# rosielab/emojivoice

Hardware: AMD Instinct MI355X
Metric: audio_seconds_per_second (higher is better)
Workload: dtype f32 (deep layers: operand = two block-scaled fp16 pieces, product = 3 fp16 products on the fp16 MFMA, f32 accumulate); 1 GPU; config2: batch 64 x 516-frame (5.99 s) utterances per GPU, 10 Euler steps + HiFi-GAN V1, 22.05 kHz; global_batch=64, frames=516, ode_steps=10, parallelism=dp1, collective=none, batch_pipeline=cfm(i+1) || hifigan(i) on two streams, 2 pipeline(s) in flight

## Files before the change

emojivoice_amd/_lib.py:

```python
from __future__ import annotations

import ctypes as C
import math
import os
import subprocess
from typing import Dict, Optional

import numpy as np
import torch

_HERE = os.path.dirname(os.path.abspath(__file__))
LIB_PATH = os.environ.get("EV_LIB_PATH") or os.path.join(_HERE, "lib", "libemojivoice_hip.so")
CSRC = os.path.join(_HERE, "csrc")
SOURCES = [os.path.join(CSRC, n) for n in ("ev_engine.hip", "ev_kernels.h", "ev_analysis_kernels.h", "ev_analysis.h")] \
    + [os.path.join(os.path.dirname(_HERE), "include", "emojivoice.h")]

EXPORTS = [
    "ev_abi_version", "ev_create", "ev_destroy", "ev_last_error", "ev_load_estimator", "ev_load_vocoder", "ev_load_vocoder_cfg", "ev_load_text_encoder", "ev_text_encoder",
    "ev_text_encoder_status", "ev_stft_magnitude", "ev_denoise", "ev_align", "ev_dbg_conv_bench",
    "ev_workspace_bytes", "ev_cfm_decode", "ev_estimator", "ev_hifigan", "ev_profile_enable", "ev_profile_read", "ev_profile_read_split", "ev_dbg_last_cfg", "ev_set_arithmetic", "ev_get_arithmetic",
    "ev_op_conv1d", "ev_op_groupnorm_mish", "ev_op_groupnorm_mish2", "ev_op_conv_groupnorm", "ev_op_layernorm", "ev_op_split_pieces", "ev_op_attention", "ev_op_ln_mlp", "ev_set_mrf_streams_max",
    "ev_cfm_decode2", "ev_reserve", "ev_alloc_count", "ev_dbg_sk_stats", "ev_op_attn_out", "ev_dbg_set_amax", "ev_dbg_set_attn_h16", "ev_dbg_set_chain", "ev_dbg_sk_taken",
    "ev_load_mel_basis", "ev_mel_spectrogram",
    "ev_maximum_path", "ev_log_prior", "ev_mas_align",
    "ev_estimator_rows", "ev_cfm_loss",
    "ev_load_resampler", "ev_resample", "ev_mel_stats",
    "ev_trim_bounds", "ev_trim_apply",
    "ev_pitch_yin", "ev_dtw",
    "ev_loudness",
    "ev_pyin_observe", "ev_pyin_decode",
    "ev_op_attention2", "ev_op_attn_out2",
    "ev_load_stoi", "ev_stoi",
    "ev_load_stft_dist", "ev_stft_dist",
    "ev_load_voice_quality", "ev_voice_quality",
    "ev_load_formants", "ev_formants", "ev_formant_track",
    "ev_perturbation",
    "ev_load_harmonics", "ev_harmonics",
    "ev_functionals", "ev_modulation",
    "ev_load_auditory", "ev_auditory",
    "ev_load_srmr", "ev_srmr",
    "ev_load_speech_rate", "ev_speech_rate",
    "ev_load_envelope", "ev_envelope",
    "ev_load_phase_vocoder", "ev_phase_vocoder",
    "ev_op_conv1d_epi",
]


class EvLibraryError(RuntimeError):
    pass


class ev_tensor_index(C.Structure):
    _fields_ = [("name", C.c_char_p), ("offset", C.c_uint64), ("ndim", C.c_int32), ("shape", C.c_int64 * 4)]


# ... 118 lines not shown
    lib.ev_stft_dist.argtypes = [vp, vp, vp, vp, i32, i32, C.c_double, vp, vp, vp, vp]
    lib.ev_load_voice_quality.argtypes = [vp, vp, vp, i32, i32, i32, vp, vp, i32, i32, i32, vp, C.c_double]
    lib.ev_voice_quality.argtypes = [vp, vp, vp, i32, i32, C.c_double, vp, vp, vp, vp]
    lib.ev_load_formants.argtypes = [vp, vp, i32, i32, i32, C.c_double, C.c_double, C.c_double, i32]
    lib.ev_formants.argtypes = [vp, vp, vp, i32, i32, C.c_double, vp, vp, vp, vp]
    lib.ev_formant_track.argtypes = [vp, vp, vp, i32, i32, i32, i32, vp, C.c_double, C.c_double, C.c_double, vp, vp, vp, vp, vp]
    lib.ev_perturbation.argtypes = [vp, vp, vp, i32, i32, i32, vp, i32, i32, C.c_double, C.c_double, C.c_double, vp, vp, vp, vp]
    lib.ev_load_harmonics.argtypes = [vp, vp, vp, i32, i32, i32, C.c_double, i32, C.c_double, C.c_double, C.c_double]
    lib.ev_harmonics.argtypes = [vp, vp, vp, i32, i32, vp, vp, vp, i32, C.c_double, vp, vp, vp, vp]
    lib.ev_functionals.argtypes = [vp, vp, vp, vp, i32, i32, i32, vp, i32, vp, vp, vp]
    lib.ev_modulation.argtypes = [vp, vp, vp, vp, i32, i32, i32, C.c_double, C.c_double, i32, i32, C.c_double, vp, i32, vp, vp, vp, vp, vp, vp]
    lib.ev_load_auditory.argtypes = [vp, vp, vp, i32, i32, i32, vp, i32, vp, vp, i32, i32, i32, C.c_double]
    lib.ev_auditory.argtypes = [vp, vp, vp, i32, i32, C.c_double, vp, vp, vp, vp, vp]
    lib.ev_load_srmr.argtypes = [vp, vp, vp, vp, vp, vp, i32, i32, i32]
    lib.ev_srmr.argtypes = [vp, vp, vp, i32, i32, vp, vp, vp, vp, vp]
    lib.ev_load_speech_rate.argtypes = [vp, vp, i32, i32]
    lib.ev_speech_rate.argtypes = [vp, vp, vp, vp, i32, i32, C.c_double, C.c_double, C.c_double, C.c_double, i32, i32, vp, vp, vp, vp, vp]
    lib.ev_load_envelope.argtypes = [vp, vp, i32, i32, C.c_double, C.c_double, C.c_double, vp, i32]
    lib.ev_envelope.argtypes = [vp, vp, vp, vp, i32, i32, C.c_double, vp, vp, vp, vp]
    lib.ev_load_phase_vocoder.argtypes = [vp, vp, vp, i32]
    lib.ev_phase_vocoder.argtypes = [vp, vp, vp, i32, i32, C.c_double, vp, i32, vp, vp, vp, vp]
    lib.ev_maximum_path.argtypes = [vp, vp, vp, vp, i32, i32, i32, vp, vp, vp]
    lib.ev_log_prior.argtypes = [vp, vp, vp, i32, i32, i32, vp, vp]
    lib.ev_mas_align.argtypes = [vp, vp, vp, vp, vp, i32, i32, i32, vp, vp, vp, vp, vp]
    lib.ev_profile_enable.argtypes = [vp, i32]
    lib.ev_profile_read.argtypes = [vp, C.POINTER(C.c_double), C.POINTER(C.c_double), C.POINTER(C.c_int64), i32]
    lib.ev_profile_read_split.argtypes = [vp, C.POINTER(C.c_double), C.POINTER(C.c_double), C.POINTER(C.c_int64)]
    lib.ev_dbg_last_cfg.argtypes = [vp]
    lib.ev_set_arithmetic.argtypes = [vp, i32]
    lib.ev_get_arithmetic.argtypes = [vp]
    lib.ev_dbg_set_amax.argtypes = [vp, i32]
    lib.ev_dbg_set_attn_h16.argtypes = [vp, i32]
    lib.ev_dbg_set_chain.argtypes = [vp, i32]
    lib.ev_dbg_sk_taken.argtypes = [vp]
    lib.ev_dbg_sk_taken.restype = C.c_int64
    lib.ev_op_conv1d.argtypes = [vp, vp, vp, vp, i32, i32, i32, i32, i32, i32, i32, i32, i32, f32, vp, vp]
    lib.ev_op_conv1d_epi.argtypes = [vp, vp, vp, vp, i32, i32, i32, i32, i32, i32, i32, i32, i32, i32, C.POINTER(ev_conv_epi), vp, vp, vp, vp]
    lib.ev_op_groupnorm_mish.argtypes = [vp, vp, vp, vp, vp, i32, i32, i32, i32, vp, vp]
    lib.ev_op_groupnorm_mish2.argtypes = [vp, vp, vp, vp, vp, i32, i32, i32, i32, i32, vp, i32, vp, vp, vp]
    lib.ev_op_conv_groupnorm.argtypes = [vp, vp, vp, vp, i32, i32, i32, vp, vp, vp, i32, vp, vp, vp, vp, vp, C.POINTER(C.c_int), vp]
    lib.ev_op_layernorm.argtypes = [vp, vp, vp, vp, i32, i32, vp, vp]
    lib.ev_op_split_pieces.argtypes = [vp, vp, i32, vp, vp]
    lib.ev_op_attention.argtypes = [vp, vp, vp, i32, i32, i32, vp, vp]
    lib.ev_op_attn_out.argtypes = [vp, vp, vp, i32, i32, vp, vp, vp, vp]
    lib.ev_op_attention2.argtypes = [vp, vp, vp, i32, i32, i32, i32, i32, i32, vp, C.POINTER(C.c_int), vp]
    lib.ev_op_attn_out2.argtypes = [vp, vp, vp, i32, i32, i32, i32, vp, vp, f32, f32, f32, vp, C.POINTER(C.c_int), vp]
    lib.ev_op_ln_mlp.argtypes = [vp, vp, vp, vp, vp, vp, vp, vp, vp, vp, vp, i32, i32, i32, vp, vp]
    for n in EXPORTS:
        getattr(lib, n)
    _lib = lib
    return lib


def _stream_ptr() -> int:
    return int(torch.cuda.current_stream().cuda_stream)


def _ptr(t):
    return None if t is None else t.data_ptr()


class Engine:

    def __init__(self, device: int = 0, spk_emb_dim: int = 64, heads: int = 2):
        if not torch.cuda.is_available():
            raise EvLibraryError("no ROCm GPU visible: the EmojiVoice hot path has no CPU fallback")
# ... 781 lines not shown
        B, F, T = mel.shape
        assert F == 80
        wav = torch.empty((B, 1, T * 256), dtype=torch.float32, device=mel.device)
        per_utt = (T + 2 * self.voc_pad0) * self.voc_frame_bytes
        bmax = max(1, int((2**32 - 2**20) // per_utt))
        for b0 in range(0, B, bmax):
            b1 = min(B, b0 + bmax)
            self._check(self.lib.ev_hifigan(self.h, mel[b0:b1].data_ptr(), b1 - b0, T, wav[b0:b1].data_ptr(), _stream_ptr()), "ev_hifigan")
        return wav

    def workspace_bytes(self, B: int, Tp: int, Tv: int) -> int:
        return int(self.lib.ev_workspace_bytes(self.h, B, Tp, Tv))

    def profile_enable(self, on: bool):
        self._check(self.lib.ev_profile_enable(self.h, int(on)), "ev_profile_enable")

    def op_split_pieces(self, x):
        x = self._f32(x).reshape(-1)
        out = torch.empty((3, x.numel()), dtype=torch.float32, device=x.device)
        self._check(self.lib.ev_op_split_pieces(self.h, x.data_ptr(), x.numel(), out.data_ptr(), _stream_ptr()), "ev_op_split_pieces")
        return out

    def set_arithmetic(self, bf16_products: int):
        self._check(self.lib.ev_set_arithmetic(self.h, int(bf16_products)), "ev_set_arithmetic")

    def set_amax(self, on: bool) -> None:
        self._check(self.lib.ev_dbg_set_amax(self.h, int(bool(on))), "ev_dbg_set_amax")

    def set_attn_h16(self, on: bool) -> None:
        self._check(self.lib.ev_dbg_set_attn_h16(self.h, int(bool(on))), "ev_dbg_set_attn_h16")

    def set_chain(self, on: bool) -> None:
        self._check(self.lib.ev_dbg_set_chain(self.h, int(bool(on))), "ev_dbg_set_chain")

    def arithmetic(self) -> int:
        return int(self.lib.ev_get_arithmetic(self.h))

    def last_cfg(self) -> int:
        return int(self.lib.ev_dbg_last_cfg(self.h))

    def profile_read_split(self):
        ms, fl, n = C.c_double(), C.c_double(), C.c_int64()
        self._check(self.lib.ev_profile_read_split(self.h, C.byref(ms), C.byref(fl), C.byref(n)), "ev_profile_read_split")
        return ms.value, fl.value, n.value

    def profile_read(self, reset: bool = True):
        ms, fl, n = C.c_double(), C.c_double(), C.c_int64()
        self._check(self.lib.ev_profile_read(self.h, C.byref(ms), C.byref(fl), C.byref(n), int(reset)), "ev_profile_read")
        return ms.value, fl.value, n.value

    def op_conv1d(self, x, w, bias, dilation=1, transposed=False, stride=1, padding=0, pre_lrelu_slope=-1.0):
        x = self._f32(x)
        B, Cin, T = x.shape
        w = np.ascontiguousarray(w.detach().cpu().float().numpy())
        if transposed:
            Cout, K = w.shape[1], w.shape[2]
            Tout = T * stride
        else:
            Cout, K = w.shape[0], w.shape[2]
            Tout = T // stride
        bp = None
        if bias is not None:
            bnp = np.ascontiguousarray(bias.detach().cpu().float().numpy())
            bp = bnp.ctypes.data_as(C.c_void_p)
        y = torch.empty((B, Cout, Tout), dtype=torch.float32, device=x.device)
        self._check(self.lib.ev_op_conv1d(self.h, x.data_ptr(), w.ctypes.data_as(C.c_void_p), bp, B, Cin, T, Cout, K, dilation,
# ... 163 lines not shown
```

emojivoice_amd/csrc/ev_engine.hip:

```cpp
#include "ev_kernels.h"
#include "../../include/emojivoice.h"

#include <math.h>
#include <stdlib.h>
#include <stdarg.h>
#include <stdio.h>
#include <string.h>

#include <algorithm>
#include <atomic>
#include <mutex>
#include <numeric>
#include <string>
#include <unordered_map>
#include <vector>

namespace {

struct HostTensor {
    const float* p = nullptr;
    int ndim = 0;
    int64_t shape[4] = {0, 0, 0, 0};
    int64_t numel() const { int64_t n = 1; for (int i = 0; i < ndim; ++i) n *= shape[i]; return n; }
};
// ... 102 lines not shown
    ResamplerW rs;
    StoiW stoi;
    StftDistW stftd;
    VoiceQW voiceq;
    FormantW fmt;
    HarmW harm;
    AudW aud;
    SrmrW srmr;
    RateW rate;
    EnvW env;
    PvW pv;
    struct Scratch { char* p = nullptr; size_t bytes = 0; hipStream_t last = nullptr; bool last_valid = false; };
    Scratch dn_ws, enc_ws, mas_ws;
    Scratch dtw_ws;
    Scratch stat_ws;
    Scratch trim_ws;
    Scratch loud_ws;
    Scratch stoi_ws;
    Scratch stftd_ws;
    Scratch srmr_ws;
    Scratch rate_ws;
    Scratch env_ws;
    Scratch pv_ws;
    float* zeros = nullptr;
    int max_steps = 64;
    int* bad_ids_host = nullptr; int* bad_ids_dev = nullptr;
    char* ws = nullptr; size_t ws_bytes = 0; size_t ws_used = 0; size_t ws_bytes_last = 0;
    int ws_B = -1, ws_Tp = -1, ws_Tv = -1;
    bool prof = false;
    bool fuse_pairs = true;
    bool fuse_attn = true;
    bool attn_h16 = true;
    bool use_chain = true;
    bool fuse_mlp = true;
    int gn_stats_tiles = 0;
    int fuse_mlp_min_tiles = 96;
    std::vector<hipEvent_t> ev_pool; size_t ev_used = 0;
    hipStream_t ws_stream = nullptr; bool ws_stream_valid = false;
    float* temb_host[2] = {nullptr, nullptr}; size_t temb_cap[2] = {0, 0}; hipEvent_t temb_ev[2] = {nullptr, nullptr}; int temb_slot = 0;
    float* cap_pool = nullptr; size_t cap_stride = 0; int cap_used = 0; int cap_nt[8] = {0};
    struct TprojEntry { int nt; float* d; };
    std::vector<TprojEntry> tproj_cache;
    bool captured = false; int cap_B = 0, cap_Tp = 0;
    int64_t n_allocs = 0;
    double prof_flops = 0; int64_t prof_launches = 0;
    struct ProfRec { int kind, Cin, Cout, ntaps, nrows, cfg, lean; double flops; bool split = false; };
    std::vector<ProfRec> prof_recs;
    hipStream_t stream = nullptr;
    hipStream_t mrf_stream[2] = {nullptr, nullptr};
    hipEvent_t mrf_ev[4] = {nullptr, nullptr, nullptr, nullptr};
    int ncu = 0;
    unsigned* sk_ctrl = nullptr;
    unsigned sk_seq = 0;
    float* sk_part = nullptr;
    int split_terms = 16;
    bool use_amax = true;
    bool amax_emitted = false;
    int n_fp32_only_layers = 0;
    int last_cfg = -1;
    bool sk_balance = true;
    int sk_wgs = 2;
    int sk_spin = 3000;
    int mrf_max_frames = 16384;
    int force_cfg = -1;
    bool lean = true;
    bool small_sk = true;
// ... 805 lines not shown
    const ConvLayer& Lout = mode == 0 ? *L2 : L1;
    p.Y = Y; p.ldy = ldy; p.Cout = Lout.Cout; p.bias = mode == 0 ? Lout.bias : nullptr; p.osplit_log2 = 31; p.isplit_log2 = 31; p.mmul = 1;
    p.nrows = g.nrows; p.S = g.S; p.P = g.P; p.T = g.T; p.scale = 1.f;
    p.R = R; p.ldr = 256; p.rowmask = rowmask; p.mask2 = (mode == 0 && rowmask) ? 1 : 0;
    mp.X = X; mp.ldx = 256; mp.ln_g = ln_g; mp.ln_b = ln_b; mp.ln_eps = 1e-5f;
    if (!L1.bias && !h->zeros) {
        HIPCHK(h, hipMalloc((void**)&h->zeros, 4096 * sizeof(float)));
        HIPCHK(h, hipMemsetAsync(h->zeros, 0, 4096 * sizeof(float), h->stream));
        h->owned.push_back(h->zeros);
    }
    if (L1.Mpad > 4096) return fail(h, "launch_mlp: hidden width %d > 4096", L1.Mpad);
    mp.W1 = L1.W; mp.b1 = L1.bias ? L1.bias : h->zeros; mp.M1 = L1.Mpad; mp.alpha = alpha; mp.binv = binv; mp.W2 = L2 ? L2->W : nullptr;
    if (L1.Cin != 256 || L1.Kpad != 256 || L1.ntaps != 1 || (L1.Mpad % 128) || L1.Cout != L1.Mpad || (ldy & 3))
        return fail(h, "launch_mlp: first linear must be 256 -> multiple of 128 (got %d -> %d)", L1.Cin, L1.Cout);
    if (mode == 0 && (!L2 || L2->Cout != 256 || L2->Mpad != 256 || L2->Cin != L1.Cout || L2->Kpad != L1.Mpad || L2->ntaps != 1 || !L2->bias || !alpha || !binv))
        return fail(h, "launch_mlp: second linear must be %d -> 256 with bias", L1.Cout);
    if (over_4gib(g, std::max(ldy, 256))) return fail(h, "tensor exceeds the 4 GiB buffer-addressing limit: split the batch");
    if (g.S < 4 && g.nrows > 1) return fail(h, "launch_mlp: utterance stride %d < 4 rows is not supported by the lean row walk", g.S);
    const int nchunk = L1.Mpad / 128;
    const double flops = 2.0 * (L1.macs_per_row + (L2 ? L2->macs_per_row : 0.0)) * valid_rows(g);
    {
        const int split_terms = h->split_terms;
        const int nt64 = (g.nrows + 63) / 64;
        if (mode == 0 && (split_terms == 6 || split_terms == 16) && L1.Wx && L2->Wx && h->sk_balance && h->ncu > 0 && h->ncu <= EV_SK_MAXWG && nt64 >= h->ncu) {
            const int grid = h->ncu;
            const bool h16 = split_terms == 16 && L1.Wh && L2->Wh;
            mp.W1x = L1.Wx; mp.W2x = L2->Wx; mp.ntiles = nt64;
            mp.W1h = L1.Wh; mp.W2h = L2->Wh; mp.w1_scale = L1.wh_scale; mp.w2_scale = L2->wh_scale;
            if (sk_setup(h, mp.sk, (long)nt64 * nchunk, grid, h16)) return 1;
            if (L1.Mpad > 1024) return fail(h, "launch_mlp: hidden width %d > 1024 (LDS table of the SnakeBeta vectors)", L1.Mpad);
            const size_t smem = h16 ? (size_t)64 * (4 * 256 + 16) + (size_t)64 * (4 * 128 + 16) + 16 + (size_t)2 * L1.Mpad * sizeof(float) + 64
                                    : (size_t)64 * (6 * 256 + 16) + (size_t)64 * (6 * 128 + 16) + 16 + (size_t)2 * L1.Mpad * sizeof(float);
            if (prof_begin(h)) return 1;
            if (h16) launch<ln_mlp_h16_kernel<0>>(h->device, dim3(grid), dim3(256), smem, h->stream, mp);
            else launch<ln_mlp_split_kernel<6>>(h->device, dim3(grid), dim3(256), smem, h->stream, mp);
            HIPCHK(h, hipGetLastError());
            return h->prof ? prof_end(h, {2, 256, Lout.Cout, 1, g.nrows, h16 ? 121 : 120, 1, flops, true}) : 0;
        }
    }
    {
        const int nt64 = (g.nrows + 63) / 64;
        if (mode == 1 && h->split_terms == 16 && h->qkv_h16 && L1.Wh && L1.Mpad == 384 && !R && !rowmask && h->ncu > 0 && nt64 >= h->ncu) {
            mp.W1h = L1.Wh; mp.w1_scale = L1.wh_scale; mp.ntiles = nt64;
            if (qkv_scale && qkv_packed && qkv_scale[0] > 0.f && qkv_scale[1] > 0.f && qkv_scale[2] > 0.f) {
                mp.qkv_pack = 1; *qkv_packed = 1;
                for (int i = 0; i < 3; ++i) mp.qkv_scale[i] = qkv_scale[i];
            }
            const size_t smem = (size_t)64 * (4 * 256 + 16) + 32;
            if (prof_begin(h)) return 1;
            launch<ln_qkv_h16_kernel<0>>(h->device, dim3(nt64), dim3(256), smem, h->stream, mp);
            HIPCHK(h, hipGetLastError());
            h->last_cfg = 122;
            return h->prof ? prof_end(h, {3, 256, Lout.Cout, 1, g.nrows, 122, 1, flops, true}) : 0;
        }
    }
    const int ntiles = (g.nrows + 31) / 32;
    size_t smem = (size_t)(32 * 260 + 4 * 32 * 36 + 4) * sizeof(float);
    int grid = ntiles;
    mp.ntiles = ntiles;
    mp.sk.q = nchunk; mp.sk.r = 0; mp.sk.spin_limit = h->sk_spin;
    const int wpc = h->sk_wgs;
    const bool big = ntiles >= h->ncu && (long)ntiles * nchunk >= (long)wpc * h->ncu;
    if (h->sk_balance && h->ncu > 0 && wpc * h->ncu <= EV_SK_MAXWG && big) {
        const long U = (long)ntiles * nchunk;
        grid = (int)std::min<long>((long)wpc * h->ncu, U);
        if (sk_setup(h, mp.sk, U, grid, false)) return 1;
        if (wpc != 2) smem = std::max(smem, (size_t)((160 * 1024 / wpc) & ~255));
    }
    if (prof_begin(h)) return 1;
// ... 663 lines not shown
        constexpr int w = decltype(kernel_tag)::value;
        if (fused) launch<mas_search_kernel<w, true>>(h->device, dim3(B), dim3(NT), smem, st, p);
        else launch<mas_search_kernel<w, false>>(h->device, dim3(B), dim3(NT), smem, st, p);
    };
    dispatch<16, 4>(W, go);
    HIPCHK(h, hipGetLastError());
    if (d_attn || d_mu_y) {
        hipLaunchKernelGGL(mas_fill_kernel, dim3((Ty + 255) / 256, B, d_attn ? (Tx + 63) / 64 : 1), dim3(256), 0, st, (const int32_t*)p.idx, d_mu_x, d_attn, d_mu_y, C, Tx, Ty);
        HIPCHK(h, hipGetLastError());
    }
    return 0;
}

}

extern "C" {

int ev_abi_version(void) { return EV_ABI_VERSION; }

int ev_create(ev_handle** out, int device, const ev_model_dims* dims) {
    if (!out || !dims) return 1;
    *out = nullptr;
    int ndev = 0;
    if (hipGetDeviceCount(&ndev) != hipSuccess || device < 0 || device >= ndev) return 2;
    if (hipSetDevice(device) != hipSuccess) return 3;
    ev_handle* h = new ev_handle();
    h->device = device;
    h->dims = *dims;
    { const char* fp = getenv("EV_FUSE_PAIRS"); if (fp && *fp == '0') h->fuse_pairs = false; }
    { const char* fp = getenv("EV_FUSE_MLP"); if (fp && *fp == '0') h->fuse_mlp = false; }
    { const char* fp = getenv("EV_FUSE_ATTN"); if (fp && *fp == '0') h->fuse_attn = false; }
    if (getenv("EV_NO_ATTN_H16")) h->attn_h16 = false;
    if (getenv("EV_NO_CHAIN")) h->use_chain = false;
    { const char* fp = getenv("EV_FUSE_MLP_MIN"); if (fp && *fp) h->fuse_mlp_min_tiles = atoi(fp); }
    { const char* fp = getenv("EV_MRF_STREAMS_MAX"); if (fp && *fp) h->mrf_max_frames = atoi(fp); }
    if (getenv("EV_NO_AMAX")) h->use_amax = false;
    { const char* sp = getenv("EV_SPLIT"); if (sp && *sp) { const int t = atoi(sp); h->split_terms = (t == 0 || t == 3 || t == 6 || t == 9 || t == 16) ? t : 16; } }
    { const char* fp = getenv("EV_NO_SK_BALANCE"); if (fp && *fp && *fp != '0') h->sk_balance = false; }
    { const char* fp = getenv("EV_SK_SPIN"); if (fp && *fp) h->sk_spin = atoi(fp); }
    { const char* fp = getenv("EV_SK_WGS"); if (fp && *fp) h->sk_wgs = std::min(3, std::max(1, atoi(fp))); }
    { const char* fp = getenv("EV_FORCE_CFG"); if (fp && *fp) h->force_cfg = atoi(fp); }
    if (getenv("EV_NO_LEAN")) h->lean = false;
    if (getenv("EV_NO_SK")) h->small_sk = false;
    if (getenv("EV_NO_SK32_LEAN")) h->sk32_lean = false;
    if (getenv("EV_NO_GN_STATS")) h->gn_stats = false;
    if (getenv("EV_NO_QKV_H16")) h->qkv_h16 = false;
    if (getenv("EV_NO_ATTN_SK")) h->attn_sk = false;
    { const char* fp = getenv("EV_ATTN_TPW"); if (fp) h->attn_tpw = std::max(1, atoi(fp)); }
    if (getenv("EV_FULL_REZERO")) h->full_rezero = true;
    { const char* fp = getenv("EV_RB2_MINKEEP"); if (fp) h->rb2_minkeep = atoi(fp); }
    if (hipDeviceGetAttribute(&h->ncu, hipDeviceAttributeMultiprocessorCount, device) != hipSuccess) h->ncu = 0;
    if (dims->n_feats != 80 || dims->channels != 256 || dims->head_dim != 64 || dims->heads != 2) {
        delete h;
        return 4;
    }
    *out = h;
    return 0;
}

void ev_destroy(ev_handle* h) {
    if (!h) return;
    hipSetDevice(h->device);
    hipDeviceSynchronize();
    for (void* p : h->owned) hipFree(p);
    if (h->ws) hipFree(h->ws);
    if (h->cap_pool) hipHostFree(h->cap_pool);
// ... 942 lines not shown
    if (reset) { h->ev_used = 0; h->prof_flops = 0; h->prof_launches = 0; h->prof_recs.clear(); }
    return 0;
}

int ev_dbg_last_cfg(ev_handle* h) { return h ? h->last_cfg : -1; }

int ev_set_arithmetic(ev_handle* h, int bf16_products) {
    if (!h) return 1;
    if (bf16_products != 0 && bf16_products != 3 && bf16_products != 6 && bf16_products != 9 && bf16_products != 16)
        return fail(h, "ev_set_arithmetic: 0, 3, 6, 9 or 16, got %d", bf16_products);
    h->split_terms = bf16_products;
    return 0;
}
int ev_get_arithmetic(ev_handle* h) { return h ? h->split_terms : -1; }

int ev_dbg_set_amax(ev_handle* h, int on) {
    if (!h) return 1;
    h->use_amax = on != 0;
    return 0;
}

int ev_dbg_set_chain(ev_handle* h, int on) {
    if (!h) return 1;
    h->use_chain = on != 0;
    return 0;
}

int ev_dbg_set_attn_h16(ev_handle* h, int on) {
    if (!h) return 1;
    h->attn_h16 = on != 0;
    return 0;
}

int ev_profile_read_split(ev_handle* h, double* ms_out, double* flops_out, int64_t* launches_out) {
    if (!h) return 1;
    HIPCHK(h, hipStreamSynchronize(h->stream));
    double ms = 0, fl = 0;
    int64_t n = 0;
    if (h->prof_recs.size() * 2 == h->ev_used)
        for (size_t i = 0; i < h->prof_recs.size(); ++i) {
            const auto& r = h->prof_recs[i];
            if (!r.split) continue;
            float t = 0;
            HIPCHK(h, hipEventElapsedTime(&t, h->ev_pool[2 * i], h->ev_pool[2 * i + 1]));
            ms += t; fl += r.flops; n += 1;
        }
    if (ms_out) *ms_out = ms;
    if (flops_out) *flops_out = fl;
    if (launches_out) *launches_out = n;
    return 0;
}

int ev_dbg_conv_bench(ev_handle* h, int Cin, int Cout, int K, int dil, int B, int T, int P, int iters, int dbg, int cfg, float* ms_out) {
    const int stagger = (dbg & 64) ? 0 : -1;
    const bool planar = (dbg & 32) != 0;
    const bool no_res = (dbg & 128) != 0;
    const bool no_pro = (dbg & 512) != 0;
    dbg &= ~(64 | 32 | 128 | 512);
    if (enter(h)) return 1;
    h->stream = nullptr;
    std::vector<float> w((size_t)Cout * Cin * K), b(Cout);
    unsigned s = 12345u;
    for (auto& v : w) { s = s * 1664525u + 1013904223u; v = ((s >> 8) * (1.0f / 16777216.0f) - 0.5f) * 0.1f; }
    for (auto& v : b) { s = s * 1664525u + 1013904223u; v = ((s >> 8) * (1.0f / 16777216.0f) - 0.5f); }
    HostTensor wt, bt;
    wt.p = w.data(); wt.ndim = 3; wt.shape[0] = Cout; wt.shape[1] = Cin; wt.shape[2] = K;
// ... 500 lines not shown
```

emojivoice_amd/csrc/ev_kernels.h:

```cpp
#pragma once
#include <hip/hip_runtime.h>
#include <stdint.h>
#include <type_traits>

typedef float f32x16 __attribute__((ext_vector_type(16)));
typedef float f32x4 __attribute__((ext_vector_type(4)));
typedef int i32x4 __attribute__((ext_vector_type(4)));

#define EV_MAX_TAPS 16
#define EV_BK 32
#define EV_LDK 36
#define EV_WROWS 128
#define EV_SK_MAXF4(TW) ((TW) == 4 ? (64 + 64) * 8 * 8 : 16 * 512)
#define EV_HALO 64

enum { ACT_NONE = 0, ACT_LRELU = 1, ACT_TANH = 2, ACT_SILU = 3, ACT_MISH = 4, ACT_SNAKE = 5 };

struct SkCtl {
    unsigned* ctrl;
    unsigned* flags;
    float* part;
    int part_floats;
    int q, r;
    int spin_limit;
// ... 3977 lines not shown
            while (c1 < nchunk) {
                int n = 0;
                while (n < 64 && gi + n < (int)gridDim.x && sk_start(mp.sk, gi + n) < tile_end) ++n;
                if (n == 0) break;
                const int ready = sk_wait_many(mp.sk, gi, n, tag, tid, skw);
                for (int k = 0; k < ready; ++k) acc_io((unsigned)(gi + k) * pslot, 1);
                gi += ready;
                if (ready < n) {
                    const int sgi = sk_start(mp.sk, gi);
                    int egi = sk_start(mp.sk, gi + 1);
                    egi = egi < tile_end ? egi : tile_end;
                    acc_io((unsigned)g * pslot + pslot / 2, 0);
                    asm volatile("s_waitcnt vmcnt(0)" ::: "memory");
                    cA = sgi - t * nchunk; cB = egi - t * nchunk;
                    spilled = true; again = true;
                    ++gi;
                    break;
                }
            }
            if (again) {
                const int ht0 = cA * 4 + wave;
                ldP(R0, ht0, 0); ldP(R1, ht0, 1); ldP(R2, ht0, 2); ldP(R3, ht0, 3); ldP(R4, ht0, 4); ldP(R5, ht0, 5); ldP(R6, ht0, 6); ldP(R7, ht0, 7);
                continue;
            }
            conv_epilogue_lean<2, 2, 1>(p, acc2, smem + wave * (32 * 68), wave * 64, n0, lane);
            break;
        }
    }
    if (pend_pub) sk_publish(mp.sk, g, tag, tid);
    sk_arrive(mp.sk, tag, tid);
}

template <int UNUSED = 0>
__global__ __launch_bounds__(256, 2) void ln_qkv_h16_kernel(const MlpParams mp) {
    constexpr int NT = 64, C = 256, TM = 3;
    constexpr int XRS = 4 * C + 16;
    const ConvParams& p = mp.ep;
    extern __shared__ __attribute__((aligned(16))) float smem[];
    char* Xb = (char*)smem;
    float* red = (float*)(Xb + NT * XRS);
    const int tid = threadIdx.x, lane = tid & 63;
    const int wave = __builtin_amdgcn_readfirstlane(tid >> 6);
    const int li = lane & 31, lh = lane >> 5;
    const __amdgpu_buffer_rsrc_t rX = ev_rsrc(mp.X), rW1 = ev_rsrc(mp.W1h), rB1 = ev_rsrc(mp.b1);
    const unsigned wlane = (unsigned)lane * 16u;
    const int n0 = blockIdx.x * NT;
    if (ev_tile_is_padding(p.S, p.P, p.T, p.nrows, n0, NT)) return;
    f32x4 A[4][TM][2];
    auto ldA = [&](f32x4 (&dst)[TM][2], int sl) {
#pragma unroll
        for (int i = 0; i < TM; ++i)
#pragma unroll
            for (int pc = 0; pc < 2; ++pc) dst[i][pc] = ev_bload4(rW1, wlane, (unsigned)((((wave * TM + i) * (C / 16) + sl) * 2 + pc) * 1024));
    };
    ldA(A[0], 0); ldA(A[1], 1); ldA(A[2], 2);
    f32x4 bq[TM][4];
    const unsigned coff = (unsigned)(4 * lh) * 4u;
#pragma unroll
    for (int i = 0; i < TM; ++i)
#pragma unroll
        for (int q = 0; q < 4; ++q) bq[i][q] = ev_bload4(rB1, coff + (unsigned)((wave * TM + i) * 32 + 8 * q) * 4u, 0);
    float sx;
    {
        const f32x4 gm = *(const f32x4*)(mp.ln_g + lane * 4), be = *(const f32x4*)(mp.ln_b + lane * 4);
        f32x4 xv[16];
#pragma unroll
// ... 1562 lines not shown
```

include/emojivoice.h:

```cpp
#ifndef EMOJIVOICE_H
#define EMOJIVOICE_H

#include <stddef.h>
#include <stdint.h>

#ifdef __cplusplus
extern "C" {
#endif

#define EV_ABI_VERSION 4

typedef struct ev_handle ev_handle;

typedef struct ev_tensor_index {
    const char *name;
    uint64_t offset;
    int32_t ndim;
    int64_t shape[4];
} ev_tensor_index;

typedef struct ev_model_dims {
    int32_t n_feats;
    int32_t spk_emb_dim;
    int32_t channels;
// ... 173 lines not shown

int ev_functionals(ev_handle *h, const double *d_v , const uint8_t *d_mask ,
                   const int32_t *d_len , int B, int K, int F,
                   const double *q , int NQ,
                   double *d_stat , int32_t *d_count , void *stream);

int ev_modulation(ev_handle *h, const double *d_v , const uint8_t *d_mask ,
                  const int32_t *d_len , int B, int K, int F,
                  double nu0, double dnu, int NM, int min_run, double min_cycles,
                  const int32_t *band , int NBAND,
                  double *d_spec , int32_t *d_weight , double *d_peak ,
                  double *d_stat , int32_t *d_count , void *stream);

int ev_load_auditory(ev_handle *h, const double *window , const double *twiddle , int W, int H, int nfft,
                     const double *mel_w , int n_mel, const double *eq ,
                     const double *dct , int n_ceps, int k_lo, int k_hi, double compress );
int ev_auditory(ev_handle *h, const float *d_x , const int32_t *d_len , int B, int L, double power_floor,
                double *d_frame , double *d_mfcc , int32_t *d_flags ,
                double *d_bands , void *stream);

int ev_profile_enable(ev_handle *h, int on);
int ev_profile_read(ev_handle *h, double *conv_ms, double *conv_flops, int64_t *conv_launches, int reset);
int ev_profile_read_split(ev_handle *h, double *ms, double *flops, int64_t *launches);
int ev_set_arithmetic(ev_handle *h, int setting);
int ev_get_arithmetic(ev_handle *h);

int ev_dbg_last_cfg(ev_handle *h);

int ev_dbg_conv_bench(ev_handle *h, int Cin, int Cout, int K, int dil, int B, int T, int P, int iters, int dbg, int cfg, float *ms_out);

int ev_dbg_set_amax(ev_handle *h, int on);
int ev_dbg_set_attn_h16(ev_handle *h, int on);
int ev_dbg_set_chain(ev_handle *h, int on);

int ev_dbg_sk_stats(ev_handle *h, uint32_t *out3);
int64_t ev_dbg_sk_taken(ev_handle *h);

int ev_op_conv1d(ev_handle *h, const float *d_x , const float *w ,
                 const float *bias , int B, int Cin, int T, int Cout, int K, int dilation,
                 int transposed, int stride, int padding, float pre_lrelu_slope , float *d_y, void *stream);
typedef struct ev_conv_epi {
  int32_t act;
  float act_slope;
  const float *d_alpha_exp;
  const float *d_beta_inv;
  const int32_t *d_lengths;
  int32_t mask1, mask2;
  float scale;
  const float *d_R;
  int32_t accum;
  const float *d_yold;
  int32_t div3;
  float act2_slope;
  float pre_lrelu_slope;
} ev_conv_epi;
#define EV_CONV_EPI_SENTINEL 1234.5f
int ev_op_conv1d_epi(ev_handle *h, const float *d_x , const float *w , const float *bias ,
                     int B, int Cin, int T, int Cout, int K, int dilation, int transposed, int stride, int padding, int P,
                     const ev_conv_epi *ep, float *d_y, float *d_y2, float *d_ypad, void *stream);
int ev_op_groupnorm_mish(ev_handle *h, const float *d_x , const float *d_gamma, const float *d_beta,
                         const int32_t *d_lengths, int B, int C, int T, int groups, float *d_y, void *stream);
int ev_op_groupnorm_mish2(ev_handle *h, const float *d_x , const float *d_gamma, const float *d_beta,
                          const int32_t *d_lengths, int B, int C, int T, int groups, int mode, const float *d_temb,
                          int temb_stride, const float *d_R, float *d_y, void *stream);
int ev_op_conv_groupnorm(ev_handle *h, const float *d_x , const float *w ,
                         const float *bias , int Cin, int T, int K, const float *d_gamma,
// ... 24 lines not shown
```

Measured before the change: 4793 audio_s/s.

## Add 8-wave fused LayerNorm-MLP fp16 kernel splitting output columns across waves

Adds a new 512-thread (8 wave) variant of the fused LayerNorm+MLP split-fp16 kernel and makes it the default for the h16 path. Waves are arranged as 4 hidden-column groups by 2 row halves, so each wave holds a smaller second-layer accumulator (32 output columns) and the kernel keeps stream-K partial reduction. The aim is more waves per block and less per-wave register pressure, to hide latency in the deep estimator MLP. In exchange it runs one block per CU with a larger tile schedule and more barrier traffic, and it brings its own scheduling hints.

Result: no change. 4827 audio_s/s (median of 6 runs) (+0.7%).

```diff
diff --git a/emojivoice_amd/_lib.py b/emojivoice_amd/_lib.py
--- a/emojivoice_amd/_lib.py
+++ b/emojivoice_amd/_lib.py
@@ -20,7 +20,7 @@
     "ev_text_encoder_status", "ev_stft_magnitude", "ev_denoise", "ev_align", "ev_dbg_conv_bench",
     "ev_workspace_bytes", "ev_cfm_decode", "ev_estimator", "ev_hifigan", "ev_profile_enable", "ev_profile_read", "ev_profile_read_split", "ev_dbg_last_cfg", "ev_set_arithmetic", "ev_get_arithmetic",
     "ev_op_conv1d", "ev_op_groupnorm_mish", "ev_op_groupnorm_mish2", "ev_op_conv_groupnorm", "ev_op_layernorm", "ev_op_split_pieces", "ev_op_attention", "ev_op_ln_mlp", "ev_set_mrf_streams_max",
-    "ev_cfm_decode2", "ev_reserve", "ev_alloc_count", "ev_dbg_sk_stats", "ev_op_attn_out", "ev_dbg_set_amax", "ev_dbg_set_attn_h16", "ev_dbg_set_chain", "ev_dbg_sk_taken",
+    "ev_cfm_decode2", "ev_reserve", "ev_alloc_count", "ev_dbg_sk_stats", "ev_op_attn_out", "ev_dbg_set_amax", "ev_dbg_set_attn_h16", "ev_dbg_set_chain", "ev_dbg_sk_taken", "ev_dbg_set_mlp_w8",
     "ev_load_mel_basis", "ev_mel_spectrogram",
     "ev_maximum_path", "ev_log_prior", "ev_mas_align",
     "ev_estimator_rows", "ev_cfm_loss",
@@ -205,6 +205,7 @@
     lib.ev_dbg_set_amax.argtypes = [vp, i32]
     lib.ev_dbg_set_attn_h16.argtypes = [vp, i32]
     lib.ev_dbg_set_chain.argtypes = [vp, i32]
+    lib.ev_dbg_set_mlp_w8.argtypes = [vp, i32]
     lib.ev_dbg_sk_taken.argtypes = [vp]
     lib.ev_dbg_sk_taken.restype = C.c_int64
     lib.ev_op_conv1d.argtypes = [vp, vp, vp, vp, i32, i32, i32, i32, i32, i32, i32, i32, i32, f32, vp, vp]
@@ -1052,6 +1053,9 @@
 
     def set_chain(self, on: bool) -> None:
         self._check(self.lib.ev_dbg_set_chain(self.h, int(bool(on))), "ev_dbg_set_chain")
+
+    def set_mlp_w8(self, on: bool) -> None:
+        self._check(self.lib.ev_dbg_set_mlp_w8(self.h, int(bool(on))), "ev_dbg_set_mlp_w8")
 
     def arithmetic(self) -> int:
         return int(self.lib.ev_get_arithmetic(self.h))
diff --git a/emojivoice_amd/csrc/ev_engine.hip b/emojivoice_amd/csrc/ev_engine.hip
--- a/emojivoice_amd/csrc/ev_engine.hip
+++ b/emojivoice_amd/csrc/ev_engine.hip
@@ -158,6 +158,7 @@
     bool fuse_attn = true;
     bool attn_h16 = true;
     bool use_chain = true;
+    bool mlp_w8 = true;
     bool fuse_mlp = true;
     int gn_stats_tiles = 0;
     int fuse_mlp_min_tiles = 96;
@@ -1029,9 +1030,11 @@
             const size_t smem = h16 ? (size_t)64 * (4 * 256 + 16) + (size_t)64 * (4 * 128 + 16) + 16 + (size_t)2 * L1.Mpad * sizeof(float) + 64
                                     : (size_t)64 * (6 * 256 + 16) + (size_t)64 * (6 * 128 + 16) + 16 + (size_t)2 * L1.Mpad * sizeof(float);
             if (prof_begin(h)) return 1;
-            if (h16) launch<ln_mlp_h16_kernel<0>>(h->device, dim3(grid), dim3(256), smem, h->stream, mp);
+            if (h16 && h->mlp_w8) launch<ln_mlp_h16w8_kernel<0>>(h->device, dim3(grid), dim3(512), smem, h->stream, mp);
+            else if (h16) launch<ln_mlp_h16_kernel<0>>(h->device, dim3(grid), dim3(256), smem, h->stream, mp);
             else launch<ln_mlp_split_kernel<6>>(h->device, dim3(grid), dim3(256), smem, h->stream, mp);
             HIPCHK(h, hipGetLastError());
+            h->last_cfg = !h16 ? 120 : h->mlp_w8 ? 123 : 121;
             return h->prof ? prof_end(h, {2, 256, Lout.Cout, 1, g.nrows, h16 ? 121 : 120, 1, flops, true}) : 0;
         }
     }
@@ -1761,6 +1764,7 @@
     { const char* fp = getenv("EV_FUSE_ATTN"); if (fp && *fp == '0') h->fuse_attn = false; }
     if (getenv("EV_NO_ATTN_H16")) h->attn_h16 = false;
     if (getenv("EV_NO_CHAIN")) h->use_chain = false;
+    if (getenv("EV_NO_MLP_W8")) h->mlp_w8 = false;
     { const char* fp = getenv("EV_FUSE_MLP_MIN"); if (fp && *fp) h->fuse_mlp_min_tiles = atoi(fp); }
     { const char* fp = getenv("EV_MRF_STREAMS_MAX"); if (fp && *fp) h->mrf_max_frames = atoi(fp); }
     if (getenv("EV_NO_AMAX")) h->use_amax = false;
@@ -2769,6 +2773,12 @@
     return 0;
 }
 
+int ev_dbg_set_mlp_w8(ev_handle* h, int on) {
+    if (!h) return 1;
+    h->mlp_w8 = on != 0;
+    return 0;
+}
+
 int ev_profile_read_split(ev_handle* h, double* ms_out, double* flops_out, int64_t* launches_out) {
     if (!h) return 1;
     HIPCHK(h, hipStreamSynchronize(h->stream));
diff --git a/emojivoice_amd/csrc/ev_kernels.h b/emojivoice_amd/csrc/ev_kernels.h
--- a/emojivoice_amd/csrc/ev_kernels.h
+++ b/emojivoice_amd/csrc/ev_kernels.h
@@ -4033,6 +4033,337 @@
 }
 
 template <int UNUSED = 0>
+__global__ __launch_bounds__(512, 1) void ln_mlp_h16w8_kernel(const MlpParams mp) {
+    constexpr int NT = 64, C = 256, HC = 128;
+    constexpr int XRS = 4 * C + 16, HRS = 4 * HC + 16;
+    const ConvParams& p = mp.ep;
+    extern __shared__ __attribute__((aligned(16))) float smem[];
+    char* Xb = (char*)smem;
+    char* Hb = Xb + NT * XRS;
+    int* skw = (int*)(Hb + NT * HRS);
+    float* Sv = (float*)(Hb + NT * HRS + 16);
+    float* red = Sv + 2 * mp.M1;
+    const int tid = threadIdx.x, lane = tid & 63;
+    const int wave = __builtin_amdgcn_readfirstlane(tid >> 6);
+    const int hw = wave & 3, jr = wave >> 2;
+    const int li = lane & 31, lh = lane >> 5;
+    const __amdgpu_buffer_rsrc_t rX = ev_rsrc(mp.X), rW1 = ev_rsrc(mp.W1h), rW2 = ev_rsrc(mp.W2h);
+    const unsigned wlane = (unsigned)lane * 16u;
+    const int nchunk = mp.M1 / HC;
+    const int KS2 = mp.M1 / 16;
+    const int g = blockIdx.x;
+    const unsigned tag = sk_tag(mp.sk);
+    int u = sk_start(mp.sk, g);
+    const int ue = sk_start(mp.sk, g + 1);
+    const unsigned claim_prev = sk_claim_start(mp.sk, g, threadIdx.x);
+    bool first_seg = true;
+    f32x4 R0[2], R1[2], R2[2], R3[2], R4[2], R5[2], R6[2], R7[2];
+    auto ldP = [&](f32x4 (&dst)[2], int ht, int sl) {
+#pragma unroll
+        for (int pc = 0; pc < 2; ++pc) dst[pc] = ev_bload4(rW1, wlane, (unsigned)(((ht * (C / 16) + sl) * 2 + pc) * 1024));
+    };
+    const __amdgpu_buffer_rsrc_t rB1 = ev_rsrc(mp.b1);
+    auto ldN = [&](f32x4 (&dst)[2], bool q2, int hx, int i) {
+        const __amdgpu_buffer_rsrc_t rs = q2 ? rW2 : rW1;
+        const unsigned off = q2 ? (unsigned)(((wave * KS2 + hx * (HC / 16) + i) * 2) * 1024) : (unsigned)(((hx * (C / 16) + i) * 2) * 1024);
+#pragma unroll
+        for (int pc = 0; pc < 2; ++pc) dst[pc] = ev_bload4(rs, wlane, off + (unsigned)(pc * 1024));
+    };
+    {
+        float va[2], vb[2];
+#pragma unroll
+        for (int q = 0; q < 2; ++q) { const int i = q * 512 + tid; va[q] = i < mp.M1 ? mp.alpha[i] : 0.f; vb[q] = i < mp.M1 ? mp.binv[i] : 0.f; }
+#pragma unroll
+        for (int q = 0; q < 2; ++q) { const int i = q * 512 + tid; if (i < mp.M1) { Sv[i] = va[q]; Sv[mp.M1 + i] = vb[q]; } }
+    }
+    const unsigned coff = (unsigned)(4 * lh) * 4u;
+    const char* xrow = Xb + (jr * 32 + li) * XRS + 16 * lh;
+    const char* hrow = Hb + li * HRS + 16 * lh;
+    const __amdgpu_buffer_rsrc_t rPart = ev_rsrc(mp.sk.part);
+    const unsigned pslot = (unsigned)mp.sk.part_floats * 8u;
+    const unsigned pelem = (unsigned)(wave * 8) * 1024u + wlane;
+    bool pend_pub = false;
+    constexpr int PA[3] = {0, 1, 0}, PB[3] = {1, 0, 0};
+
+    while (u < ue) {
+        const int t = u / nchunk, c0 = u - t * nchunk;
+        const int c1 = (ue - u < nchunk - c0) ? c0 + (ue - u) : nchunk;
+        u += c1 - c0;
+        const int n0 = t * NT;
+        if (ev_tile_is_padding(p.S, p.P, p.T, p.nrows, n0, NT)) continue;
+        if (first_seg) {
+            first_seg = false;
+            if (c0 != 0 && sk_claim_taken(mp.sk, claim_prev, tid, skw)) continue;
+        }
+        {
+            const int ht0 = c0 * 4 + hw;
+            ldP(R0, ht0, 0); ldP(R1, ht0, 1); ldP(R2, ht0, 2); ldP(R3, ht0, 3); ldP(R4, ht0, 4); ldP(R5, ht0, 5); ldP(R6, ht0, 6); ldP(R7, ht0, 7);
+        }
+        ev_lds_barrier();
+        float sx;
+        {
+            const f32x4 gm = *(const f32x4*)(mp.ln_g + lane * 4), be = *(const f32x4*)(mp.ln_b + lane * 4);
+            f32x4 xv[8];
+#pragma unroll
+            for (int r = 0; r < 8; ++r) {
+                const int gr = n0 + wave * 8 + r;
+                xv[r] = ev_bload4(rX, ((unsigned)(gr < p.nrows ? gr : 0) * mp.ldx + lane * 4) * 4u, 0);
+            }
+            float mx = 0.f;
+#pragma unroll
+            for (int r = 0; r < 8; ++r) {
+                xv[r] = ev_ln256_row(xv[r], gm, be, mp.ln_eps);
+                mx = fmaxf(mx, evh_absmax4(xv[r]));
+            }
+#pragma unroll
+            for (int o = 32; o > 0; o >>= 1) mx = fmaxf(mx, __shfl_xor(mx, o, 64));
+            if (lane == 0) red[wave] = mx;
+            ev_lds_barrier();
+            float tmx = fmaxf(fmaxf(fmaxf(red[0], red[1]), fmaxf(red[2], red[3])), fmaxf(fmaxf(red[4], red[5]), fmaxf(red[6], red[7])));
+            if (!evh_is_finite(tmx)) {
+                mx = 0.f;
+#pragma unroll
+                for (int r = 0; r < 8; ++r) mx = fmaxf(mx, evh_absmax4_finite(xv[r]));
+#pragma unroll
+                for (int o = 32; o > 0; o >>= 1) mx = fmaxf(mx, __shfl_xor(mx, o, 64));
+                if (lane == 0) red[8 + wave] = mx;
+                ev_lds_barrier();
+                tmx = fmaxf(fmaxf(fmaxf(red[8], red[9]), fmaxf(red[10], red[11])), fmaxf(fmaxf(red[12], red[13]), fmaxf(red[14], red[15])));
+            }
+            sx = evh_scale_for(tmx);
+#pragma unroll
+            for (int r = 0; r < 8; ++r) {
+                uint2 q0v, q1v;
+                evh_split4(xv[r] * sx, q0v, q1v);
+                char* dst = Xb + (wave * 8 + r) * XRS + lane * 8;
+                *(uint2*)(dst) = q0v; *(uint2*)(dst + 2 * C) = q1v;
+            }
+        }
+        if (pend_pub) { sk_publish(mp.sk, g, tag, tid); pend_pub = false; }
+        else ev_lds_barrier();
+
+        int cA = c0, cB = c1;
+        bool spilled = false;
+        int gi = g + 1;
+        const int tile_end = (t + 1) * nchunk;
+        for (;;) {
+            const float u1 = mp.w1_scale * sx, inv1 = 1.0f / u1;
+            float cur_unit = mp.w2_scale, sh_lds = 1.f;
+            f32x16 acc2[1][2];
+#pragma unroll
+            for (int q = 0; q < 4; ++q) {
+                f32x4 bq = {0.f, 0.f, 0.f, 0.f};
+                if (p.bias && cA == 0) bq = *(const f32x4*)(p.bias + wave * 32 + 8 * q + 4 * lh) * cur_unit;
+#pragma unroll
+                for (int j = 0; j < 2; ++j)
+#pragma unroll
+                    for (int e = 0; e < 4; ++e) acc2[0][j][4 * q + e] = bq[e];
+            }
+            f32x4 bq[4];
+#pragma unroll
+            for (int q = 0; q < 4; ++q) bq[q] = ev_bload4(rB1, coff + (unsigned)((cA * 4 + hw) * 32 + 8 * q) * 4u, 0);
+            f32x4 hvs[4];
+            float hmax = 0.f;
+            f32x4 B0[2], B1[2];
+            f32x4 H0[2][2], H1[2][2];
+            auto ldBh = [&](f32x4 (&dst)[2][2], int sl) {
+#pragma unroll
+                for (int pc = 0; pc < 2; ++pc)
+#pragma unroll
+                    for (int j = 0; j < 2; ++j) dst[pc][j] = *(const f32x4*)(hrow + j * 32 * HRS + pc * (2 * HC) + sl * 32);
+            };
+            auto mma2 = [&](const f32x4 (&a)[2], const f32x4 (&b)[2][2]) {
+#pragma unroll
+                for (int tt = 0; tt < 3; ++tt)
+#pragma unroll
+                    for (int j = 0; j < 2; ++j)
+                        acc2[0][j] = __builtin_amdgcn_mfma_f32_32x32x16_f16(__builtin_bit_cast(f16x8, a[PA[tt]]), __builtin_bit_cast(f16x8, b[PB[tt]][j]), acc2[0][j], 0, 0, 0);
+            };
+            f32x16 acc1 = {}, acc1b;
+            __builtin_assume(cA < cB);
+            for (int hc = cA; hc <= cB; ++hc) {
+                const bool p1 = hc < cB, p2 = hc > cA;
+                const int ht = (p1 ? hc : cA) * 4 + hw;
+                const int htn = hc + 1 < cB ? ht + 4 : cA * 4 + hw;
+                if (p1) {
+#pragma unroll
+                    for (int q = 0; q < 4; ++q)
+#pragma unroll
+                        for (int e = 0; e < 4; ++e) { acc1[4 * q + e] = bq[q][e] * u1; acc1b[4 * q + e] = 0.f; }
+                    auto ldB = [&](f32x4 (&dst)[2], int sl) {
+#pragma unroll
+                        for (int pc = 0; pc < 2; ++pc) dst[pc] = *(const f32x4*)(xrow + pc * (2 * C) + sl * 32);
+                    };
+                    auto mma1 = [&](const f32x4 (&a)[2], const f32x4 (&b)[2]) {
+#pragma unroll
+                        for (int tt = 0; tt < 3; ++tt) {
+                            if (tt & 1) acc1b = __builtin_amdgcn_mfma_f32_32x32x16_f16(__builtin_bit_cast(f16x8, a[PA[tt]]), __builtin_bit_cast(f16x8, b[PB[tt]]), acc1b, 0, 0, 0);
+                            else acc1 = __builtin_amdgcn_mfma_f32_32x32x16_f16(__builtin_bit_cast(f16x8, a[PA[tt]]), __builtin_bit_cast(f16x8, b[PB[tt]]), acc1, 0, 0, 0);
+                        }
+                    };
+                    const int hq2 = p2 ? hc - 1 : hc;
+                    const bool nq1 = p2 || hc + 1 >= cB;
+                    const int nx1 = p2 ? hq2 : (hc + 1 < cB ? ht + 4 : hc);
+                    ldB(B0, 0);
+#define EVX_P1(RR, BC, BN_, SL, REFILL)                                                           \
+                    ldB(BN_, ((SL) + 1) & 15);                                                    \
+                    REFILL;                                                                       \
+                    mma1(RR, BC);                                                                \
+                    __builtin_amdgcn_sched_group_barrier(0x008, 1, 0);                            \
+                    __builtin_amdgcn_sched_group_barrier(0x100, 1, 0);                            \
+                    __builtin_amdgcn_sched_group_barrier(0x020, 1, 0);                            \
+                    __builtin_amdgcn_sched_group_barrier(0x008, 1, 0);                            \
+                    __builtin_amdgcn_sched_group_barrier(0x100, 1, 0);                            \
+                    __builtin_amdgcn_sched_group_barrier(0x020, 1, 0);                            \
+                    __builtin_amdgcn_sched_group_barrier(0x008, 1, 0);                            \
+                    __builtin_amdgcn_sched_barrier(0);
+                    EVX_P1(R0, B0, B1, 0, ldP(R7, ht, 7))
+                    EVX_P1(R1, B1, B0, 1, ldP(R0, ht, 8))   EVX_P1(R2, B0, B1, 2, ldP(R1, ht, 9))   EVX_P1(R3, B1, B0, 3, ldP(R2, ht, 10))
+                    EVX_P1(R4, B0, B1, 4, ldP(R3, ht, 11))  EVX_P1(R5, B1, B0, 5, ldP(R4, ht, 12))  EVX_P1(R6, B0, B1, 6, ldP(R5, ht, 13))
+                    EVX_P1(R7, B1, B0, 7, ldP(R6, ht, 14))  EVX_P1(R0, B0, B1, 8, ldP(R7, ht, 15))
+                    EVX_P1(R1, B1, B0, 9, ldN(R0, nq1, nx1, 0))   EVX_P1(R2, B0, B1, 10, ldN(R1, nq1, nx1, 1))  EVX_P1(R3, B1, B0, 11, ldN(R2, nq1, nx1, 2))
+                    EVX_P1(R4, B0, B1, 12, ldN(R3, nq1, nx1, 3))  EVX_P1(R5, B1, B0, 13, ldN(R4, nq1, nx1, 4))  EVX_P1(R6, B0, B1, 14, ldN(R5, nq1, nx1, 5))
+                    EVX_P1(R7, B1, B0, 15, ldN(R6, nq1, nx1, 6))
+#undef EVX_P1
+                    acc1 = (acc1 + acc1b) * inv1;
+                }
+                auto snake = [&](int qh) {
+                    const int q = qh >> 1, e0 = (qh & 1) * 2;
+                    const float2 saq = *(const float2*)(Sv + ht * 32 + 8 * q + 4 * lh + e0), sbq = *(const float2*)(Sv + mp.M1 + ht * 32 + 8 * q + 4 * lh + e0);
+                    const float v0 = acc1[4 * q + e0], v1 = acc1[4 * q + e0 + 1];
+                    const float h0 = fmaf(sbq.x, ev_sin2(v0 * saq.x), v0), h1 = fmaf(sbq.y, ev_sin2(v1 * saq.y), v1);
+                    hvs[q][e0] = h0; hvs[q][e0 + 1] = h1;
+                    hmax = fmaxf(hmax, fmaxf(fabsf(h0), fabsf(h1)));
+                };
+                auto phase2 = [&]() {
+                    const int hp = hc - 1;
+                    const bool nq = p1 && hc + 1 >= cB;
+                    const int nx = hc + 1 < cB ? ht + 4 : (p1 ? hc : cA * 4 + hw);
+                    {
+                        const float nu = mp.w2_scale * sh_lds, f = nu / cur_unit;
+                        cur_unit = nu;
+#pragma unroll
+                        for (int j = 0; j < 2; ++j)
+#pragma unroll
+                            for (int r = 0; r < 16; ++r) acc2[0][j][r] *= f;
+                    }
+                    ldBh(H0, 0);
+#define EVX_P2(RA, BC, BN_, SL, REFILL)                                                           \
+                    ldBh(BN_, ((SL) + 1) & 7);                                                    \
+                    REFILL;                                                                       \
+                    mma2(RA, BC);                                                                \
+                    snake(SL);                                                                    \
+                    _Pragma("unroll") for (int i_ = 0; i_ < 2; ++i_) {                            \
+                        __builtin_amdgcn_sched_group_barrier(0x008, 3, 0);                        \
+                        __builtin_amdgcn_sched_group_barrier(0x100, 2, 0);                        \
+                        __builtin_amdgcn_sched_group_barrier(0x020, 1, 0);                        \
+                        __builtin_amdgcn_sched_group_barrier(0x002, 30, 0);                       \
+                    }                                                                             \
+                    __builtin_amdgcn_sched_barrier(0);
+                    EVX_P2(R0, H0, H1, 0, ldN(R7, true, hp, 7))
+                    EVX_P2(R1, H1, H0, 1, ldN(R0, nq, nx, 0))  EVX_P2(R2, H0, H1, 2, ldN(R1, nq, nx, 1))  EVX_P2(R3, H1, H0, 3, ldN(R2, nq, nx, 2))
+                    EVX_P2(R4, H0, H1, 4, ldN(R3, nq, nx, 3))  EVX_P2(R5, H1, H0, 5, ldN(R4, nq, nx, 4))  EVX_P2(R6, H0, H1, 6, ldN(R5, nq, nx, 5))
+                    EVX_P2(R7, H1, H0, 7, ldN(R6, nq, nx, 6))
+#undef EVX_P2
+                };
+                if (p2) phase2();
+                else if (p1) {
+#pragma unroll
+                    for (int qh = 0; qh < 8; ++qh) snake(qh);
+                }
+                if (p1) {
+#pragma unroll
+                    for (int o = 32; o > 0; o >>= 1) hmax = fmaxf(hmax, __shfl_xor(hmax, o, 64));
+                    if (lane == 0) red[8 + wave] = hmax;
+                    hmax = 0.f;
+#pragma unroll
+                    for (int q = 0; q < 4; ++q) bq[q] = ev_bload4(rB1, coff + (unsigned)(htn * 32 + 8 * q) * 4u, 0);
+                    ev_lds_barrier();
+                    float hm = fmaxf(fmaxf(fmaxf(red[8], red[9]), fmaxf(red[10], red[11])), fmaxf(fmaxf(red[12], red[13]), fmaxf(red[14], red[15])));
+                    if (!evh_is_finite(hm)) {
+                        float m2 = 0.f;
+#pragma unroll
+                        for (int q = 0; q < 4; ++q) m2 = fmaxf(m2, evh_absmax4_finite(hvs[q]));
+#pragma unroll
+                        for (int o = 32; o > 0; o >>= 1) m2 = fmaxf(m2, __shfl_xor(m2, o, 64));
+                        if (lane == 0) red[wave] = m2;
+                        ev_lds_barrier();
+                        hm = fmaxf(fmaxf(fmaxf(red[0], red[1]), fmaxf(red[2], red[3])), fmaxf(fmaxf(red[4], red[5]), fmaxf(red[6], red[7])));
+                    }
+                    sh_lds = evh_scale_for(hm);
+#pragma unroll
+                    for (int q = 0; q < 4; ++q) {
+                        uint2 q0v, q1v;
+                        evh_split4(hvs[q] * sh_lds, q0v, q1v);
+                        char* dst = Hb + (jr * 32 + li) * HRS + (hw * 32 + 8 * q + 4 * lh) * 2;
+                        *(uint2*)(dst) = q0v; *(uint2*)(dst + 2 * HC) = q1v;
+                    }
+                    ev_lds_barrier();
+                }
+            }
+            {
+                const float f = 1.0f / cur_unit;
+#pragma unroll
+                for (int j = 0; j < 2; ++j)
+#pragma unroll
+                    for (int r = 0; r < 16; ++r) acc2[0][j][r] *= f;
+            }
+            auto acc_io = [&](unsigned base, int mode) {
+#pragma unroll
+                for (int j = 0; j < 2; ++j)
+#pragma unroll
+                    for (int q = 0; q < 4; ++q) {
+                        const unsigned soff = base + (unsigned)(j * 4 + q) * 1024u;
+                        if (mode == 0) {
+                            const f32x4 v = {acc2[0][j][4 * q], acc2[0][j][4 * q + 1], acc2[0][j][4 * q + 2], acc2[0][j][4 * q + 3]};
+                            ev_bstore4_sc1(rPart, pelem, soff, v);
+                        } else {
+                            const f32x4 v = ev_bload4_sc1(rPart, pelem, soff);
+#pragma unroll
+                            for (int e = 0; e < 4; ++e) acc2[0][j][4 * q + e] += v[e];
+                        }
+                    }
+            };
+            if (spilled) { acc_io((unsigned)g * pslot + pslot / 2, 1); spilled = false; }
+            if (c0 != 0) {
+                acc_io((unsigned)g * pslot, 0);
+                pend_pub = true;
+                break;
+            }
+            bool again = false;
+            while (c1 < nchunk) {
+                int n = 0;
+                while (n < 64 && gi + n < (int)gridDim.x && sk_start(mp.sk, gi + n) < tile_end) ++n;
+                if (n == 0) break;
+                const int ready = sk_wait_many(mp.sk, gi, n, tag, tid, skw);
+                for (int k = 0; k < ready; ++k) acc_io((unsigned)(gi + k) * pslot, 1);
+                gi += ready;
+                if (ready < n) {
+                    const int sgi = sk_start(mp.sk, gi);
+                    int egi = sk_start(mp.sk, gi + 1);
+                    egi = egi < tile_end ? egi : tile_end;
+                    acc_io((unsigned)g * pslot + pslot / 2, 0);
+                    asm volatile("s_waitcnt vmcnt(0)" ::: "memory");
+                    cA = sgi - t * nchunk; cB = egi - t * nchunk;
+                    spilled = true; again = true;
+                    ++gi;
+                    break;
+                }
+            }
+            if (again) {
+                const int ht0 = cA * 4 + hw;
+                ldP(R0, ht0, 0); ldP(R1, ht0, 1); ldP(R2, ht0, 2); ldP(R3, ht0, 3); ldP(R4, ht0, 4); ldP(R5, ht0, 5); ldP(R6, ht0, 6); ldP(R7, ht0, 7);
+                continue;
+            }
+            conv_epilogue_lean<1, 2, 1>(p, acc2, smem + wave * (32 * 36), wave * 32, n0, lane);
+            break;
+        }
+    }
+    if (pend_pub) sk_publish(mp.sk, g, tag, tid);
+    sk_arrive(mp.sk, tag, tid);
+}
+
+template <int UNUSED = 0>
 __global__ __launch_bounds__(256, 2) void ln_qkv_h16_kernel(const MlpParams mp) {
     constexpr int NT = 64, C = 256, TM = 3;
     constexpr int XRS = 4 * C + 16;
diff --git a/include/emojivoice.h b/include/emojivoice.h
--- a/include/emojivoice.h
+++ b/include/emojivoice.h
@@ -229,6 +229,7 @@
 int ev_dbg_set_amax(ev_handle *h, int on);
 int ev_dbg_set_attn_h16(ev_handle *h, int on);
 int ev_dbg_set_chain(ev_handle *h, int on);
+int ev_dbg_set_mlp_w8(ev_handle *h, int on);
 
 int ev_dbg_sk_stats(ev_handle *h, uint32_t *out3);
 int64_t ev_dbg_sk_taken(ev_handle *h);
```
